# Samsung/tf-fast-rnnt

Hardware: AMD Instinct MI355X
Metric: rnnt_loss_pruned_fwd_bwd_throughput (higher is better)
Workload: dtype f32; 1 GPU; c3: rnnt_loss_pruned fwd+bwd step, B=32/GPU T=1000 S=200 C=500 s_range=5, regular, full boundary, first pass rnnt_loss_simple; global_batch=32, am_pruned=broadcast view

## Files before the change

### tf-fast-rnnt_amd/csrc/capi.hip

```cpp
#include "ftr_common.h"
#ifdef FTR_DIAG
#include "../../include/ftr_diag.h"
#endif
#include <stdlib.h>
#include <string.h>

namespace ftr {
namespace {
thread_local char g_err[512] = {0};
#ifdef FTR_DIAG
int g_mi_impl = -1;
#endif

int device_ok() {
  int n = 0;
  hipError_t e = hipGetDeviceCount(&n);
  if (e != hipSuccess || n <= 0) {
    (void)hipGetLastError();
    set_error("no usable HIP device (%s); this library has no CPU path", e == hipSuccess ? "device count is 0" : hipGetErrorString(e));
    return FTR_ERR_NO_DEVICE;
  }
  return FTR_OK;
}

// ... 635 lines not shown
  if (B == 0) return FTR_OK;
  FTR_REQUIRE(gpy && prod && lm_probs && am_probs && d_am && unigram && am_dot && R && (gpx || S == 0) && (symbols || S == 0), "smoothed_logprobs_fused_bwd_am: null pointer");
  int rc = device_ok();
  if (rc != FTR_OK) return rc;
  return simple_fused_bwd_am(gpx, gpy, Scale{scale, scale_stride, scale_mul}, prod, lm_probs, am_probs, symbols, boundary, termination_symbol, combined_scale, direct_scale, unigram, am_dot, am_only_scale, R, d_am, B, T, S, C, modified, reinterpret_cast<hipStream_t>(stream));
}

int ftr_smoothed_logprobs_bwd_w_scaled_f32(const float* gpx, const float* gpy, const float* scale, int scale_stride,
                                           float scale_mul, const float* prod, const int32_t* boundary,
                                           float combined_scale, float* W, float* rsx, float* rsy, int B, int T, int S,
                                           int modified, void* stream) {
  clear_error();
  FTR_REQUIRE(B >= 0 && T >= 1 && S >= 0, "smoothed_logprobs_bwd_w_scaled: bad sizes");
  FTR_REQUIRE(scale_stride == 0 || scale_stride == 1, "smoothed_logprobs_bwd_w_scaled: scale_stride must be 0 or 1");
  if (B == 0) return FTR_OK;
  FTR_REQUIRE(gpy && prod && W && rsx && rsy && (gpx || S == 0), "smoothed_logprobs_bwd_w_scaled: null pointer");
  int rc = device_ok();
  if (rc != FTR_OK) return rc;
  return simple_logprobs_bwd_w(gpx, gpy, Scale{scale, scale_stride, scale_mul}, prod, boundary, W, rsx, rsy, combined_scale, B, T, S, modified, reinterpret_cast<hipStream_t>(stream));
}

int ftr_smoothed_logprobs_bwd_am_scaled_f32(const float* gpx, const float* gpy, const float* scale, int scale_stride,
                                            float scale_mul, const float* damp, const float* am_probs,
                                            const int32_t* symbols, const int32_t* boundary, int termination_symbol,
                                            float direct_scale, const float* unigram, const float* am_dot,
                                            float am_only_scale, float* R, float* d_am, int B, int T, int S, int C,
                                            int modified, void* stream) {
  clear_error();
  FTR_REQUIRE(B >= 0 && T >= 1 && S >= 0 && C >= 1, "smoothed_logprobs_bwd_am_scaled: bad sizes");
  FTR_REQUIRE(termination_symbol >= 0 && termination_symbol < C, "smoothed_logprobs_bwd_am_scaled: bad termination_symbol");
  FTR_REQUIRE(scale_stride == 0 || scale_stride == 1, "smoothed_logprobs_bwd_am_scaled: scale_stride must be 0 or 1");
  if (B == 0) return FTR_OK;
  FTR_REQUIRE(gpy && damp && am_probs && d_am && unigram && am_dot && R && (gpx || S == 0) && (symbols || S == 0), "smoothed_logprobs_bwd_am_scaled: null pointer");
  int rc = device_ok();
  if (rc != FTR_OK) return rc;
  return simple_logprobs_bwd_am(gpx, gpy, Scale{scale, scale_stride, scale_mul}, damp, am_probs, symbols, boundary, termination_symbol, direct_scale, unigram, am_dot, am_only_scale, R, d_am, B, T, S, C, modified, reinterpret_cast<hipStream_t>(stream));
}

int ftr_mutual_information_band_supported(int T, int S, int r) { return mi_band_supported(T, S, r); }

static int pruned_band_fwd_entry(const float* logits, const int32_t* symbols, const int32_t* ranges, const int32_t* boundary,
                                 int termination_symbol, double delay_penalty, float* lse, float* px_band, float* py_band,
                                 int B, int T, int S, int C, int r, int modified, int hat, void* stream) {
  const char* what = hat ? "hat_pruned_band_fwd" : "pruned_band_fwd";
  clear_error();
  FTR_REQUIRE(B >= 0 && T >= 1 && S >= 0 && C >= 1 && r >= 1, "%s: bad sizes", what);
  FTR_REQUIRE(!hat || C >= 2, "%s: C = %d, HAT needs a blank and at least one other symbol", what, C);
  FTR_REQUIRE(termination_symbol >= 0 && termination_symbol < C, "%s: termination_symbol %d not in [0,%d)", what, termination_symbol, C);
  if (B == 0) return FTR_OK;
  FTR_REQUIRE(logits && ranges && lse && px_band && py_band && (symbols || S == 0), "%s: null pointer", what);
  int rc = device_ok();
  if (rc != FTR_OK) return rc;
  hipStream_t st = reinterpret_cast<hipStream_t>(stream);
  rc = lse_rows(logits, lse, (size_t)B * T * r, C, termination_symbol, hat, st);
  if (rc != FTR_OK) return rc;
  return band_gather(logits, symbols, ranges, boundary, lse, termination_symbol, delay_penalty, px_band, py_band, B, T, S, C, r, modified, hat, st);
}

int ftr_pruned_band_fwd_f32(const float* logits, const int32_t* symbols, const int32_t* ranges, const int32_t* boundary,
                            int termination_symbol, double delay_penalty, float* lse, float* px_band, float* py_band,
                            int B, int T, int S, int C, int r, int modified, void* stream) {
  return pruned_band_fwd_entry(logits, symbols, ranges, boundary, termination_symbol, delay_penalty, lse, px_band, py_band, B, T, S, C, r, modified, 0, stream);
}

int ftr_hat_pruned_band_fwd_f32(const float* logits, const int32_t* symbols, const int32_t* ranges, const int32_t* boundary,
                                int termination_symbol, double delay_penalty, float* lse, float* px_band, float* py_band,
                                int B, int T, int S, int C, int r, int modified, void* stream) {
  return pruned_band_fwd_entry(logits, symbols, ranges, boundary, termination_symbol, delay_penalty, lse, px_band, py_band, B, T, S, C, r, modified, 1, stream);
}

int ftr_band_ranges_check_i32(const int32_t* ranges, const int32_t* boundary, int32_t* flags, int B, int T, int r, void* stream) {
  clear_error();
  FTR_REQUIRE(B >= 0 && T >= 0 && r >= 1, "band_ranges_check: bad sizes");
  FTR_REQUIRE(flags && (ranges || B == 0 || T == 0), "band_ranges_check: null pointer");
  int rc = device_ok();
  if (rc != FTR_OK) return rc;
  return band_ranges_check(ranges, boundary, flags, B, T, r, reinterpret_cast<hipStream_t>(stream));
}

int ftr_mutual_information_band_f32(const float* px_band, const float* py_band, const int32_t* ranges,
                                    const int32_t* boundary, float* ans, float* gx_band, float* gy_band, int B, int T,
                                    int S, int r, int modified, void* stream) {
  return ftr_mutual_information_band_ws_f32(px_band, py_band, ranges, boundary, nullptr, 0, ans, gx_band, gy_band, B, T, S, r, modified, stream);
}

size_t ftr_mutual_information_band_workspace_floats(int B, int T, int S, int r) {
  return (B < 0 || T < 1 || S < 0 || r < 1) ? 0 : mi_band_workspace_floats(B, T, S, r);
}

int ftr_mutual_information_band_ws_f32(const float* px_band, const float* py_band, const int32_t* ranges,
                                       const int32_t* boundary, float* workspace, size_t workspace_floats, float* ans,
                                       float* gx_band, float* gy_band, int B, int T, int S, int r, int modified,
                                       void* stream) {
  clear_error();
  FTR_REQUIRE(B >= 0 && T >= 1 && S >= 0 && r >= 1, "mutual_information_band: bad sizes");
  if (B == 0) return FTR_OK;
  FTR_REQUIRE(px_band && py_band && ranges && ans && gx_band && gy_band, "mutual_information_band: null pointer");
  int rc = device_ok();
  if (rc != FTR_OK) return rc;
  return mi_band(px_band, py_band, ranges, boundary, workspace, workspace_floats, ans, gx_band, gy_band, B, T, S, r, modified, reinterpret_cast<hipStream_t>(stream));
}

static int pruned_band_bwd_scaled_entry(const float* logits, const int32_t* symbols, const int32_t* ranges,
                                        const int32_t* boundary, int termination_symbol, const float* lse,
                                        const float* gx_band, const float* gy_band, const float* scale, int scale_stride,
                                        float scale_mul, float* glogits, int B, int T, int S, int C, int r, int modified,
                                        int hat, void* stream) {
  const char* what = hat ? "hat_pruned_band_bwd_scaled" : "pruned_band_bwd_scaled";
  clear_error();
// ... 282 lines not shown
```

### tf-fast-rnnt_amd/csrc/ftr_common.h

```cpp
#pragma once
#include <hip/hip_runtime.h>
#include <stdint.h>
#include <stdio.h>
#include <stdarg.h>
#include "../../include/ftr.h"

namespace ftr {

void set_error(const char* fmt, ...);
void clear_error();

inline int check_launch(const char* what) {
  hipError_t e = hipGetLastError();
  if (e != hipSuccess) {
    set_error("%s: launch failed: %s", what, hipGetErrorString(e));
    return FTR_ERR_LAUNCH;
  }
  return FTR_OK;
}

inline int require_rows_32bit(const char* what, size_t rows) {
  if (rows > 0x7fffffffull) {
    set_error("%s: %zu rows (B*T*s_range) exceed the 2^31 - 1 that the launch grids index", what, rows);
    return FTR_ERR_INVALID_ARG;
// ... 95 lines not shown
  *sp = xb >= 0.0f ? big : small;
  *sn = xb >= 0.0f ? small : big;
}

}

namespace ftr {
int mi_plain_fwd(const float* px, const float* py, const int32_t* boundary, float* p, float* ans, int B, int S, int T, int modified, hipStream_t st);
int mi_plain_bwd(const float* px, const float* py, const int32_t* boundary, const float* p, float* p_grad, float* px_grad, float* py_grad, float* ans_grad, int overwrite, int B, int S, int T, int modified, hipStream_t st);
int mi_bidir_fwd(const float* px, const float* py, const int32_t* boundary, float* ws, size_t ws_floats, int flags, float* ans, int B, int S, int T, int modified, hipStream_t st);
int mi_bidir_bwd(const int32_t* boundary, const float* ws, size_t ws_floats, int flags, float* px_grad, float* py_grad, float* ans_grad, int overwrite, int B, int S, int T, int modified, hipStream_t st, const float* ans = nullptr, float* loss_out = nullptr, int loss_code = 0);
int mi_bidir_ws_init(float* ws, size_t ws_floats, int B, int S, int T, hipStream_t st);
int mi_bidir_status(const float* ws, size_t ws_floats, int B, int S, int T, int* status_host, long long* dirty_host, hipStream_t st);
size_t mi_bidir_workspace_floats(int B, int S, int T);
size_t mi_bidir_handoff_floats(int B, int S, int T);
size_t mi_viterbi_workspace_bytes(int B, int S, int T);
int mi_viterbi(const float* px, const float* py, const int32_t* boundary, void* ws, size_t ws_bytes, float* score, int32_t* frames, int B, int S, int T, int modified, hipStream_t st);
size_t mi_multiblank_workspace_floats(int B, int S, int T);
int mi_multiblank_fwd(const float* px, const float* py, const int32_t* boundary, const int32_t* durations, int D, float* ws, size_t ws_floats, float* ans, int B, int S, int T, hipStream_t st);
int mi_multiblank_bwd(const float* px, const float* py, const int32_t* boundary, const int32_t* durations, int D, float* ws, size_t ws_floats, const float* ans_grad, float* px_grad, float* py_grad, int B, int S, int T, hipStream_t st);
int multiblank_logprobs_fwd(const float* logits, const int32_t* symbols, const int32_t* ranges, const int32_t* boundary, int blank, const int32_t* big_ids, const int32_t* durations, int D, double sigma, double delay_penalty, float* lse, float* px, float* py, int B, int T, int S, int C, int r, hipStream_t st);
int multiblank_logprobs_bwd(const float* logits, const int32_t* symbols, const int32_t* ranges, const int32_t* boundary, int blank, const int32_t* big_ids, const int32_t* durations, int D, const float* lse, const float* gpx, const float* gpy, Scale scale, float* glogits, int B, int T, int S, int C, int r, hipStream_t st);
size_t mi_tdt_workspace_floats(int B, int S, int T);
int mi_tdt_fwd(const float* px, const float* py, const int32_t* boundary, const int32_t* token_durations, int Dx, const int32_t* blank_durations, int Dy, float* ws, size_t ws_floats, float* ans, int B, int S, int T, hipStream_t st);
int mi_tdt_bwd(const float* px, const float* py, const int32_t* boundary, const int32_t* token_durations, int Dx, const int32_t* blank_durations, int Dy, float* ws, size_t ws_floats, const float* ans_grad, float* px_grad, float* py_grad, int B, int S, int T, hipStream_t st);
int tdt_logprobs_fwd(const float* logits, const int32_t* symbols, const int32_t* ranges, const int32_t* boundary, int blank, const int32_t* durations, int N, double sigma, double delay_penalty, float* lse_tok, float* lse_dur, float* px, float* py, int B, int T, int S, int C, int r, hipStream_t st);
int tdt_logprobs_bwd(const float* logits, const int32_t* symbols, const int32_t* ranges, const int32_t* boundary, int blank, const int32_t* durations, int N, const float* lse_tok, const float* lse_dur, const float* gpx, const float* gpy, Scale scale, float* glogits, int B, int T, int S, int C, int r, hipStream_t st);
int cummin_i32(const int32_t* in, int32_t* out, int rows, int cols, hipStream_t st);
int prune_ranges(const float* px_grad, const float* py_grad, const int32_t* boundary, int32_t* ranges, int32_t* s_begin, int B, int S, int T, int T1, int r, hipStream_t st);
int do_pruning(const float* am, const float* lm, const int32_t* ranges, float* am_p, float* lm_p, int B, int T, int S1, int C, int r, hipStream_t st);
size_t do_pruning_bwd_workspace_bytes(int B, int T, int S1, int C, int r);
int do_pruning_bwd_ws(const float* g_am_p, const float* g_lm_p, const int32_t* ranges, float* d_am, float* d_lm, int B, int T, int S1, int C, int r, void* ws, size_t ws_bytes, hipStream_t st);
int do_pruning_bwd(const float* g_am_p, const float* g_lm_p, const int32_t* ranges, float* d_am, float* d_lm, int B, int T, int S1, int C, int r, hipStream_t st);
int pruned_logprobs_fwd(const float* logits, const int32_t* symbols, const int32_t* ranges, const int32_t* boundary, int blank, double delay_penalty, float* lse, float* px, float* py, int B, int T, int S, int C, int r, int modified, int hat, hipStream_t st);
int pruned_logprobs_bwd(const float* logits, const int32_t* symbols, const int32_t* ranges, const int32_t* boundary, int blank, const float* lse, const float* gpx, const float* gpy, Scale scale, float* glogits, int B, int T, int S, int C, int r, int modified, int hat, hipStream_t st);
int simple_rowmax_exp(const float* x, float* probs, float* rowmax, float* rowsum, const float* dotvec, float* dot, size_t rows, int C, hipStream_t st);
int simple_rowmax_exp_pair(const float* x1, float* probs1, float* rowmax1, size_t rows1, const float* x2, float* probs2, float* rowmax2, size_t rows2, int C, hipStream_t st);
int simple_rowdot(const float* x, const float* v, float* dot, size_t rows, int C, hipStream_t st);
size_t simple_colsum_workspace_floats(size_t rows, int C);
int simple_colsum_weighted(const float* x, const float* w, float* out, float* ws, size_t ws_floats, size_t rows, int C, hipStream_t st);
int simple_logprobs_fwd(const float* am, const float* lm, const int32_t* symbols, const float* prod, const float* am_max, const float* lm_max, const int32_t* boundary, int blank, double delay_penalty, const float* lmonly_norm, const float* amonly_norm, const float* ulog, float cs, float ls, float as, float* px, float* py, int B, int T, int S, int C, int modified, hipStream_t st);
int simple_logprobs_bwd_w(const float* gpx, const float* gpy, Scale scale, const float* prod, const int32_t* boundary, float* W, float* rsx, float* rsy, float cs, int B, int T, int S, int modified, hipStream_t st);
int simple_logprobs_bwd_am(const float* gpx, const float* gpy, Scale scale, const float* damp, const float* am_probs, const int32_t* symbols, const int32_t* boundary, int blank, float kdir, const float* uvec, const float* amdot, float as, float* Rout, float* d_am, int B, int T, int S, int C, int modified, hipStream_t st);
int simple_logprobs_bwd_lm(const float* dlmp, const float* lm_probs, const int32_t* symbols, const float* rsx, const float* rsy, int blank, float kdir, const float* arow, const float* invsum, const float* gu, float* d_lm, int B, int S, int C, hipStream_t st);
int simple_fused_supported(int C);
int simple_fused_bwd_supported(int T, int C);
int normalizer_gemm(int kind, const float* x, const float* y, float* out, int B, int T, int S1, int C, hipStream_t st);
int normalizer_gemm_choice(int kind, int B, int T, int S1, int C, int* solution, float* us, float* us_default, int* candidates);
int normalizer_gemm_set_choice(int kind, int B, int T, int S1, int C, int solution);
int simple_fused_fwd(const float* am, const float* lm, const int32_t* symbols, const float* am_probs, const float* lm_probs, const float* am_max, const float* lm_max, const int32_t* boundary, int blank, double delay_penalty, const float* lmonly_norm, const float* amonly_norm, const float* ulog, float cs, float ls, float as, float* px, float* py, float* prod_out, int B, int T, int S, int C, int modified, hipStream_t st);
int simple_fused_bwd_am(const float* gpx, const float* gpy, Scale scale, const float* prod, const float* lm_probs, const float* am_probs, const int32_t* symbols, const int32_t* boundary, int blank, float cs, float kdir, const float* uvec, const float* amdot, float as, float* Rout, float* d_am, int B, int T, int S, int C, int modified, hipStream_t st);
int negated_reduce(const float* ans, int B, int reduction, float* out, hipStream_t st);
int lse_rows(const float* logits, float* lse, size_t rows, int C, int blank, int hat, hipStream_t st);
int mi_band_supported(int T, int S, int r);
int band_ranges_check(const int32_t* ranges, const int32_t* boundary, int* flags, int B, int T, int r, hipStream_t st);
int band_gather(const float* logits, const int32_t* symbols, const int32_t* ranges, const int32_t* boundary, const float* lse, int blank, double delay_penalty, float* pxb, float* pyb, int B, int T, int S, int C, int r, int modified, int hat, hipStream_t st);
size_t mi_band_workspace_floats(int B, int T, int S, int r);
int mi_band_seg_supported(int T, int S, int r);
size_t mi_band_seg_workspace_floats(int B, int T, int S, int r);
int mi_band_seg(const float* pxb, const float* pyb, const int32_t* ranges, const int32_t* boundary, float* ws, size_t ws_floats, float* ans, float* gxb, float* gyb, int B, int T, int S, int r, int modified, hipStream_t st);
int mi_band(const float* pxb, const float* pyb, const int32_t* ranges, const int32_t* boundary, float* ws, size_t ws_floats, float* ans, float* gxb, float* gyb, int B, int T, int S, int r, int modified, hipStream_t st);
int band_grad_banded(const float* logits, const int32_t* symbols, const int32_t* ranges, const int32_t* boundary, int blank, const float* lse, const float* gxb, const float* gyb, Scale scale, float* glogits, int B, int T, int S, int C, int r, int modified, int hat, hipStream_t st);
int selftest(hipStream_t st, int* result_dev);
int debug_stamps(unsigned long long* out16);
int debug_trace(unsigned long long* out, int n);
}
```

### tf-fast-rnnt_amd/csrc/prune.hip

```cpp
#include "ftr_common.h"
#include <cstdlib>
#include <limits.h>

namespace ftr {
namespace {

__device__ __forceinline__ int wave_incl_min_scan(int v, int lane) {
#pragma unroll
  for (int off = 1; off < 64; off <<= 1) {
    const int t = __shfl_up(v, off, 64);
    if (lane >= off) v = min(v, t);
  }
  return v;
}

__global__ void cummin_kernel(const int32_t* __restrict__ in, int32_t* __restrict__ out, int rows, int cols) {
  const int lane = threadIdx.x & 63;
  const int row = blockIdx.x * (blockDim.x >> 6) + (threadIdx.x >> 6);
  if (row >= rows) return;
  const int32_t* src = in + (size_t)row * cols;
  int32_t* dst = out + (size_t)row * cols;
  int carry = INT_MAX;
  for (int c0 = 0; c0 < cols; c0 += 64) {
    const int c = c0 + lane;
// ... 147 lines not shown
  int best = 0;
  float bestv = 0.0f;
  float nv[2][CHK], xv[2][CHK];
  auto fetch = [&](int c0, float (&n)[CHK], float (&x)[CHK]) {
#pragma unroll
    for (int u = 0; u < CHK; ++u) {
      const int s0 = c0 + u;
      n[u] = (s0 + 1 < nwin) ? pyc[(size_t)(s0 + R) * T] : 0.0f;
      x[u] = (s0 > 0 && s0 < nwin) ? pxc[(size_t)(s0 - 1) * T1] : 0.0f;
    }
  };
  auto consume = [&](int c0, const float (&n)[CHK], const float (&x)[CHK]) {
#pragma unroll
    for (int u = 0; u < CHK; ++u) {
      const int s0 = c0 + u;
      const float g = (u < R) ? carry[u < R ? u : 0] : n[u >= R ? u - R : 0];
      if (s0 < nwin) {
        const float blk = lead - lag;
        const float fin = blk - x[u];
        if (s0 == 0 || fin > bestv) { best = s0; bestv = fin; }
        if (s0 + 1 < nwin) {
          lead = lead + n[u];
          lag = lag + g;
        }
      }
    }
#pragma unroll
    for (int i = 0; i < R; ++i) carry[i] = n[CHK - R + i];
  };
  fetch(0, nv[0], xv[0]);
  for (int c0 = 0; c0 < nwin; c0 += 2 * CHK) {
    if (c0 + CHK < nwin) fetch(c0 + CHK, nv[1], xv[1]);
    consume(c0, nv[0], xv[0]);
    if (c0 + CHK < nwin) {
      if (c0 + 2 * CHK < nwin) fetch(c0 + 2 * CHK, nv[0], xv[0]);
      consume(c0 + CHK, nv[1], xv[1]);
    }
  }
  const int se = boundary[4 * b + 2], te = boundary[4 * b + 3];
  int pad = se - R + 1;
  if (pad < 0) pad = 0;
  s_begin[(size_t)b * T + t] = (t < te - 1) ? best : pad;
}

__device__ __forceinline__ int wave_incl_suffix_min(int v, int lane) {
#pragma unroll
  for (int off = 1; off < 64; off <<= 1) {
    const int t = __shfl_down(v, off, 64);
    if (lane + off < 64) v = min(v, t);
  }
  return v;
}

__global__ void prune_adjust_kernel(const int32_t* __restrict__ s_begin, int32_t* __restrict__ ranges, int B,
                                    int T, int r_out, int r_con) {
  const int lane = threadIdx.x & 63;
  const int b = blockIdx.x * (blockDim.x >> 6) + (threadIdx.x >> 6);
  if (b >= B) return;
  constexpr int PER = 16, SB = 64 * PER;
  const int32_t* x = s_begin + (size_t)b * T;
  int carry1 = INT_MAX, carry2 = INT_MAX;
  for (int base = ((T - 1) / SB) * SB; base >= 0; base -= SB) {
    const int t0 = base + lane * PER;
    int v[PER];
#pragma unroll
    for (int i = 0; i < PER; ++i) v[i] = (t0 + i < T) ? x[t0 + i] : INT_MAX;
#pragma unroll
    for (int i = PER - 2; i >= 0; --i) v[i] = min(v[i], v[i + 1]);
    int incl = wave_incl_suffix_min(v[0], lane);
    int right = __shfl_down(incl, 1, 64);
    right = (lane == 63) ? carry1 : min(right, carry1);
    carry1 = min(__shfl(incl, 0, 64), carry1);
#pragma unroll
    for (int i = 0; i < PER; ++i) {
      const int t = t0 + i;
      v[i] = (t < T) ? -(min(v[i], right) - (r_con - 1) * t) : INT_MAX;
    }
#pragma unroll
    for (int i = PER - 2; i >= 0; --i) v[i] = min(v[i], v[i + 1]);
    incl = wave_incl_suffix_min(v[0], lane);
    right = __shfl_down(incl, 1, 64);
    right = (lane == 63) ? carry2 : min(right, carry2);
    carry2 = min(__shfl(incl, 0, 64), carry2);
#pragma unroll
    for (int i = 0; i < PER; ++i) {
      const int t = t0 + i;
      if (t < T) {
        const int z = max(min(v[i], right), 0);
        const int sb = -(z - (r_con - 1) * t);
        int32_t* dst = ranges + ((size_t)b * T + t) * r_out;
        for (int k = 0; k < r_out; ++k) dst[k] = sb + k;
      }
    }
  }
}

template <bool VEC>
__global__ __launch_bounds__(128) void do_pruning_kernel(const float* __restrict__ am, const float* __restrict__ lm,
                                                         const int32_t* __restrict__ ranges, float* __restrict__ am_p,
                                                         float* __restrict__ lm_p, int T, int S1, int C, int r) {
  const bool copy_am = am_p != nullptr;
  size_t bt = blockIdx.x;
  if ((gridDim.x & 7u) == 0) bt = (size_t)(blockIdx.x & 7u) * (gridDim.x >> 3) + (blockIdx.x >> 3);
  const size_t b = bt / T;
  const int32_t* rg = ranges + bt * r;
  const float* lmb = lm + b * S1 * C;
  float* ao = am_p + bt * r * C;
  float* lo = lm_p + bt * r * C;
  if (VEC) {
    const int n4 = C >> 2;
    const f4u* arow = reinterpret_cast<const f4u*>(am + bt * C);
    for (int c4 = threadIdx.x; c4 < n4; c4 += 128) {
      f4 a = {0.0f, 0.0f, 0.0f, 0.0f};
      if (copy_am) a = arow[c4];
      for (int k0 = 0; k0 < r; k0 += 8) {
        f4 l[8];
#pragma unroll
        for (int u = 0; u < 8; ++u)
          if (k0 + u < r) l[u] = reinterpret_cast<const f4u*>(lmb + (size_t)min(max(rg[k0 + u], 0), S1 - 1) * C)[c4];
#pragma unroll
        for (int u = 0; u < 8; ++u)
          if (k0 + u < r) {
            if (copy_am) __builtin_nontemporal_store(a, reinterpret_cast<f4u*>(ao + (size_t)(k0 + u) * C) + c4);
            __builtin_nontemporal_store(l[u], reinterpret_cast<f4u*>(lo + (size_t)(k0 + u) * C) + c4);
          }
      }
    }
  } else {
    for (int c = threadIdx.x; c < C; c += 128) {
      const float a = copy_am ? am[bt * C + c] : 0.0f;
      for (int k = 0; k < r; ++k) {
        if (copy_am) ao[(size_t)k * C + c] = a;
        lo[(size_t)k * C + c] = lmb[(size_t)min(max(rg[k], 0), S1 - 1) * C + c];
      }
    }
  }
}

template <bool VEC>
__global__ void do_pruning_bwd_am_kernel(const float* __restrict__ g_am_p, float* __restrict__ d_am, int C, int r,
                                         size_t total) {
  const int per_row = VEC ? (C >> 2) : C;
  for (size_t i = (size_t)blockIdx.x * blockDim.x + threadIdx.x; i < total; i += (size_t)gridDim.x * blockDim.x) {
    const size_t bt = i / per_row;
    const int c = (int)(i - bt * per_row);
// ... 392 lines not shown
  const int threads = 256;
  if ((C & 3) == 0) {
    const size_t total = (size_t)B * T * (C >> 2);
    hipLaunchKernelGGL(do_pruning_bwd_am_kernel<true>, dim3((unsigned)((total + threads - 1) / threads)), dim3(threads), 0, st, g_am_p, d_am, C, r, total);
  } else {
    const size_t total = (size_t)B * T * C;
    hipLaunchKernelGGL(do_pruning_bwd_am_kernel<false>, dim3((unsigned)((total + threads - 1) / threads)), dim3(threads), 0, st, g_am_p, d_am, C, r, total);
  }
  int rc = check_launch("do_pruning_bwd_am");
  if (rc != FTR_OK) return rc;
  const size_t lds = sizeof(int) * (size_t)T * r;
  if (lds > 150 * 1024) { set_error("do_pruning_bwd: T*s_range = %d too large for the LDS row list", T * r); return FTR_ERR_UNSUPPORTED; }
  const bool vec = (C & 3) == 0;
  if (lds > 64 * 1024) {
    hipError_t e = vec ? hipFuncSetAttribute(reinterpret_cast<const void*>(do_pruning_bwd_lm_kernel<true>), hipFuncAttributeMaxDynamicSharedMemorySize, (int)lds)
                       : hipFuncSetAttribute(reinterpret_cast<const void*>(do_pruning_bwd_lm_kernel<false>), hipFuncAttributeMaxDynamicSharedMemorySize, (int)lds);
    if (e != hipSuccess) { set_error("do_pruning_bwd: cannot reserve LDS: %s", hipGetErrorString(e)); return FTR_ERR_LAUNCH; }
  }
  if (vec) hipLaunchKernelGGL(do_pruning_bwd_lm_kernel<true>, dim3(S1, B), dim3(64), lds, st, g_lm_p, ranges, d_lm, T, S1, C, r);
  else hipLaunchKernelGGL(do_pruning_bwd_lm_kernel<false>, dim3(S1, B), dim3(64), lds, st, g_lm_p, ranges, d_lm, T, S1, C, r);
  return check_launch("do_pruning_bwd_lm");
}

int cummin_i32(const int32_t* in, int32_t* out, int rows, int cols, hipStream_t st) {
  if (rows == 0 || cols == 0) return FTR_OK;
  const int waves_per_block = 4;
  hipLaunchKernelGGL(cummin_kernel, dim3((rows + waves_per_block - 1) / waves_per_block),
                     dim3(64 * waves_per_block), 0, st, in, out, rows, cols);
  return check_launch("cummin_i32");
}

int prune_ranges(const float* px_grad, const float* py_grad, const int32_t* boundary, int32_t* ranges,
                 int32_t* s_begin, int B, int S, int T, int T1, int r, hipStream_t st) {
  if (B == 0 || T == 0) return FTR_OK;
  const int threads = 64;
  const dim3 grid((T + threads - 1) / threads, B);
#define FTR_ARGMAX_ONCE(R) case R: hipLaunchKernelGGL(prune_argmax_once_kernel<R>, grid, dim3(threads), 0, st, px_grad, py_grad, boundary, s_begin, B, S, T, T1); break;
  const int nwin = S + 1 - r + 1;
  if (nwin > ftr::kSplitQ && (size_t)((T + 63) / 64) * B <= 768) {
    const int nc = (nwin + ftr::kSplitQ - 1) / ftr::kSplitQ;
    const int nw = nc < 8 ? nc : 8;
    hipLaunchKernelGGL(prune_argmax_split_kernel, dim3((T + 63) / 64, B), dim3(64 * nw), 0, st, px_grad, py_grad, boundary, s_begin, B, S, T, T1, r);
  } else
  switch (r) {
    FTR_ARGMAX_ONCE(1) FTR_ARGMAX_ONCE(2) FTR_ARGMAX_ONCE(3) FTR_ARGMAX_ONCE(4) FTR_ARGMAX_ONCE(5) FTR_ARGMAX_ONCE(6)
    FTR_ARGMAX_ONCE(7) FTR_ARGMAX_ONCE(8) FTR_ARGMAX_ONCE(9) FTR_ARGMAX_ONCE(10) FTR_ARGMAX_ONCE(11) FTR_ARGMAX_ONCE(12)
    FTR_ARGMAX_ONCE(13) FTR_ARGMAX_ONCE(14) FTR_ARGMAX_ONCE(15) FTR_ARGMAX_ONCE(16)
    default: hipLaunchKernelGGL(prune_argmax_kernel, grid, dim3(threads), 0, st, px_grad, py_grad, boundary, s_begin, B, S, T, T1, r);
  }
#undef FTR_ARGMAX_ONCE
  int rc = check_launch("prune_argmax");
  if (rc != FTR_OK) return rc;
  const int r_con = (T1 == T) ? 2 : r;
  hipLaunchKernelGGL(prune_adjust_kernel, dim3(B), dim3(64), 0, st, s_begin, ranges, B, T, r, r_con);
  return check_launch("prune_adjust");
}

int do_pruning(const float* am, const float* lm, const int32_t* ranges, float* am_p, float* lm_p, int B, int T, int S1,
               int C, int r, hipStream_t st) {
  const size_t frames = (size_t)B * T;
  if (frames == 0 || C == 0 || r == 0) return FTR_OK;
  { const int rc32 = require_rows_32bit("do_pruning", frames * (size_t)r); if (rc32 != FTR_OK) return rc32; }
  if ((C & 3) == 0) hipLaunchKernelGGL(do_pruning_kernel<true>, dim3((unsigned)frames), dim3(128), 0, st, am, lm, ranges, am_p, lm_p, T, S1, C, r);
  else hipLaunchKernelGGL(do_pruning_kernel<false>, dim3((unsigned)frames), dim3(128), 0, st, am, lm, ranges, am_p, lm_p, T, S1, C, r);
  return check_launch("do_pruning");
}

size_t do_pruning_bwd_workspace_bytes(int B, int T, int S1, int C, int r) {
  if ((C & 3) != 0 || (size_t)B * T * C == 0 || r <= 0) return 0;
  const int seg = ftr::seg_frames(B, T);
  const size_t nseg = (size_t)(T + seg - 1) / seg;
  const size_t partial = sizeof(float) * (size_t)B * nseg * (2 * (size_t)r) * C;
  return partial + sizeof(int4) * (size_t)B * nseg;
}

int do_pruning_bwd_ws(const float* g_am_p, const float* g_lm_p, const int32_t* ranges, float* d_am, float* d_lm,
                      int B, int T, int S1, int C, int r, void* ws, size_t ws_bytes, hipStream_t st) {
  if ((size_t)B * T * C == 0) return FTR_OK;
  if ((C & 3) != 0 || r <= 0) return do_pruning_bwd(g_am_p, g_lm_p, ranges, d_am, d_lm, B, T, S1, C, r, st);
  const size_t need = do_pruning_bwd_workspace_bytes(B, T, S1, C, r);
  if (!ws || ws_bytes < need || (reinterpret_cast<uintptr_t>(ws) & 15) != 0) {
    set_error("do_pruning_bwd_ws: workspace of %zu bytes (16-byte aligned) required, got %zu", need, ws_bytes);
    return FTR_ERR_INVALID_ARG;
  }
  const int seg = ftr::seg_frames(B, T);
  const int nseg = (T + seg - 1) / seg;
  float* partial = reinterpret_cast<float*>(ws);
  int4* meta = reinterpret_cast<int4*>(partial + (size_t)B * nseg * (2 * (size_t)r) * C);
  const size_t lds = sizeof(int) * (size_t)seg;
  if (r > ftr::kSegMaxR || lds > 60 * 1024 || (size_t)B * nseg * (2 * (size_t)r) >= 0x7fffffffull || (size_t)B * T * r >= 0x7fffffffull)
    return do_pruning_bwd(g_am_p, g_lm_p, ranges, d_am, d_lm, B, T, S1, C, r, st);
  const bool fuse = (g_am_p == g_lm_p);
  if (!fuse) {
    const size_t total = (size_t)B * T * (C >> 2);
    hipLaunchKernelGGL(ftr::do_pruning_bwd_am_kernel<true>, dim3((unsigned)((total + 255) / 256)), dim3(256), 0, st, g_am_p, d_am, C, r, total);
    int rc = check_launch("do_pruning_bwd_am");
    if (rc != FTR_OK) return rc;
  }
#define FTR_SEG(R) case R: \
    if (fuse) hipLaunchKernelGGL((ftr::do_pruning_bwd_seg_kernel<R, true>), dim3(nseg, B), dim3(128), lds, st, g_lm_p, ranges, d_am, d_lm, partial, meta, T, S1, C, seg); \
    else hipLaunchKernelGGL((ftr::do_pruning_bwd_seg_kernel<R, false>), dim3(nseg, B), dim3(128), lds, st, g_lm_p, ranges, d_am, d_lm, partial, meta, T, S1, C, seg); \
    break;
  switch (r) {
    FTR_SEG(1) FTR_SEG(2) FTR_SEG(3) FTR_SEG(4) FTR_SEG(5) FTR_SEG(6) FTR_SEG(7) FTR_SEG(8)
    FTR_SEG(9) FTR_SEG(10) FTR_SEG(11) FTR_SEG(12) FTR_SEG(13) FTR_SEG(14) FTR_SEG(15) FTR_SEG(16)
  }
#undef FTR_SEG
// ... 9 lines not shown
```

### tf-fast-rnnt_amd/csrc/pruned_logprobs.hip

```cpp
#include "ftr_common.h"

namespace ftr {
namespace {

__device__ __forceinline__ float wave_max(float v) { return wave_max_dpp(v); }
__device__ __forceinline__ float wave_sum(float v) { return wave_sum_dpp(v); }

template <int NQ, bool HAT>
__global__ __launch_bounds__(256) void lse_rows_reg_kernel(const float* __restrict__ logits, float* __restrict__ lse,
                                                           size_t rows, int C, int blank) {
  const int lane = threadIdx.x & 63;
  const size_t rowi = (size_t)blockIdx.x * (blockDim.x >> 6) + (threadIdx.x >> 6);
  if (rowi >= rows) return;
  const size_t row = rows - 1 - rowi;
  const int n4 = C >> 2;
  const f4 ninf = {-INFINITY, -INFINITY, -INFINITY, -INFINITY};
  const f4u* x4 = reinterpret_cast<const f4u*>(logits + row * C);
  f4 v[NQ];
#pragma unroll
  for (int q = 0; q < NQ; ++q) {
    const int i = lane + 64 * q;
    v[q] = (i < n4) ? (f4)x4[i] : ninf;
    if (HAT) {
#pragma unroll
      for (int e = 0; e < 4; ++e) v[q][e] = (4 * i + e == blank) ? -INFINITY : v[q][e];
    }
  }
  float m = -INFINITY;
#pragma unroll
  for (int q = 0; q < NQ; ++q) m = fmaxf(fmaxf(m, fmaxf(v[q][0], v[q][1])), fmaxf(v[q][2], v[q][3]));
  m = wave_max(m);
  float sum = 0.0f;
#pragma unroll
  for (int q = 0; q < NQ; ++q) {
    if (lane + 64 * q < n4)
      sum += __expf(v[q][0] - m) + __expf(v[q][1] - m) + __expf(v[q][2] - m) + __expf(v[q][3] - m);
  }
  sum = wave_sum(sum);
  if (lane == 0) lse[row] = m + __logf(sum);
}

template <bool VEC, bool HAT>
__global__ void lse_rows_kernel(const float* __restrict__ logits, float* __restrict__ lse, size_t rows, int C, int blank) {
  const int lane = threadIdx.x & 63;
  const size_t row = (size_t)blockIdx.x * (blockDim.x >> 6) + (threadIdx.x >> 6);
  if (row >= rows) return;
  const float* x = logits + row * C;
  float m = -INFINITY;
  if (VEC) {
    const f4u* x4 = reinterpret_cast<const f4u*>(x);
    const int n4 = C >> 2;
    for (int i = lane; i < n4; i += 64) {
      f4 v = x4[i];
      if (HAT) {
#pragma unroll
        for (int e = 0; e < 4; ++e) v[e] = (4 * i + e == blank) ? -INFINITY : v[e];
      }
      m = fmaxf(fmaxf(m, fmaxf(v[0], v[1])), fmaxf(v[2], v[3]));
    }
    m = wave_max(m);
    float s = 0.0f;
    for (int i = lane; i < n4; i += 64) {
      f4 v = x4[i];
      if (HAT) {
#pragma unroll
        for (int e = 0; e < 4; ++e) v[e] = (4 * i + e == blank) ? -INFINITY : v[e];
      }
      s += __expf(v[0] - m) + __expf(v[1] - m) + __expf(v[2] - m) + __expf(v[3] - m);
    }
    s = wave_sum(s);
    if (lane == 0) lse[row] = m + __logf(s);
  } else {
    for (int i = lane; i < C; i += 64) m = fmaxf(m, (HAT && i == blank) ? -INFINITY : x[i]);
    m = wave_max(m);
    float s = 0.0f;
    for (int i = lane; i < C; i += 64) s += __expf(((HAT && i == blank) ? -INFINITY : x[i]) - m);
    s = wave_sum(s);
    if (lane == 0) lse[row] = m + __logf(s);
  }
}

template <bool MOD, bool HAT>
__global__ void band_to_lattice_kernel(const float* __restrict__ logits, const int32_t* __restrict__ symbols,
                                       const int32_t* __restrict__ ranges, const int32_t* __restrict__ boundary,
                                       const float* __restrict__ lse, int blank, double delay_penalty,
                                       float* __restrict__ px, float* __restrict__ py, int T, int S, int C, int r) {
  const int t = blockIdx.x * blockDim.x + threadIdx.x;
  const int s = blockIdx.y, b = blockIdx.z;
  const int T1 = MOD ? T : T + 1;
  if (t >= T1 && t >= T) return;
  const int te = boundary ? boundary[4 * b + 3] : T;
  float vx = -INFINITY, vy = -INFINITY;
// ... 102 lines not shown
          val = gy * sn - gx * sp;
        } else {
          val += gy;
        }
      }
      g[c] = val;
    }
  }
}

__global__ __launch_bounds__(256) void negated_reduce_kernel(const float* __restrict__ ans, int B, int reduction,
                                                             float* __restrict__ out) {
  __shared__ float red[4];
  if (reduction == 0) {
    for (int b = threadIdx.x; b < B; b += 256) out[b] = -ans[b];
    return;
  }
  float s = 0.0f;
  for (int b = threadIdx.x; b < B; b += 256) s += ans[b];
  s = wave_sum(s);
  if ((threadIdx.x & 63) == 0) red[threadIdx.x >> 6] = s;
  __syncthreads();
  if (threadIdx.x == 0) {
    const float t = (red[0] + red[1]) + (red[2] + red[3]);
    out[0] = (reduction == 1) ? -(t / (float)B) : -t;
  }
}
}

int negated_reduce(const float* ans, int B, int reduction, float* out, hipStream_t st) {
  hipLaunchKernelGGL(negated_reduce_kernel, dim3(1), dim3(256), 0, st, ans, B, reduction, out);
  return check_launch("negated_reduce");
}

template <bool HAT>
static void lse_rows_launch(const float* logits, float* lse, size_t rows, int C, int blank, hipStream_t st) {
  const int wpb = 4;
  const unsigned blocks = (unsigned)((rows + wpb - 1) / wpb);
  if ((C & 3) == 0 && C <= 256) hipLaunchKernelGGL((lse_rows_reg_kernel<1, HAT>), dim3(blocks), dim3(64 * wpb), 0, st, logits, lse, rows, C, blank);
  else if ((C & 3) == 0 && C <= 512) hipLaunchKernelGGL((lse_rows_reg_kernel<2, HAT>), dim3(blocks), dim3(64 * wpb), 0, st, logits, lse, rows, C, blank);
  else if ((C & 3) == 0 && C <= 1024) hipLaunchKernelGGL((lse_rows_reg_kernel<4, HAT>), dim3(blocks), dim3(64 * wpb), 0, st, logits, lse, rows, C, blank);
  else if ((C & 3) == 0 && C <= 2048) hipLaunchKernelGGL((lse_rows_reg_kernel<8, HAT>), dim3(blocks), dim3(64 * wpb), 0, st, logits, lse, rows, C, blank);
  else if ((C & 3) == 0) hipLaunchKernelGGL((lse_rows_kernel<true, HAT>), dim3(blocks), dim3(64 * wpb), 0, st, logits, lse, rows, C, blank);
  else hipLaunchKernelGGL((lse_rows_kernel<false, HAT>), dim3(blocks), dim3(64 * wpb), 0, st, logits, lse, rows, C, blank);
}
int lse_rows(const float* logits, float* lse, size_t rows, int C, int blank, int hat, hipStream_t st) {
  if (rows == 0) return FTR_OK;
  { const int rc32 = require_rows_32bit("lse_rows", rows); if (rc32 != FTR_OK) return rc32; }
  if (hat) lse_rows_launch<true>(logits, lse, rows, C, blank, st);
  else lse_rows_launch<false>(logits, lse, rows, C, blank, st);
  return check_launch("lse_rows");
}

int pruned_logprobs_fwd(const float* logits, const int32_t* symbols, const int32_t* ranges,
                        const int32_t* boundary, int blank, double delay_penalty, float* lse, float* px,
                        float* py, int B, int T, int S, int C, int r, int modified, int hat, hipStream_t st) {
  const size_t rows = (size_t)B * T * r;
  if (rows == 0) return FTR_OK;
  { const int rc32 = require_rows_32bit("pruned_logprobs_fwd", rows); if (rc32 != FTR_OK) return rc32; }
  int rc = lse_rows(logits, lse, rows, C, blank, hat, st);
  if (rc != FTR_OK) return rc;
  const int threads = 256;
  const dim3 grid((T + 1 + threads - 1) / threads, S + 1, B);
#define FTR_LAUNCH_BL(MODV, HATV) hipLaunchKernelGGL((band_to_lattice_kernel<MODV, HATV>), grid, dim3(threads), 0, st, \
    logits, symbols, ranges, boundary, lse, blank, delay_penalty, px, py, T, S, C, r)
  if (modified) { if (hat) FTR_LAUNCH_BL(true, true); else FTR_LAUNCH_BL(true, false); }
  else { if (hat) FTR_LAUNCH_BL(false, true); else FTR_LAUNCH_BL(false, false); }
#undef FTR_LAUNCH_BL
  return check_launch("band_to_lattice");
}

int pruned_logprobs_bwd(const float* logits, const int32_t* symbols, const int32_t* ranges,
                        const int32_t* boundary, int blank, const float* lse, const float* gpx,
                        const float* gpy, Scale scale, float* glogits, int B, int T, int S, int C,
                        int r, int modified, int hat, hipStream_t st) {
  const size_t rows = (size_t)B * T * r;
  if (rows == 0) return FTR_OK;
  { const int rc32 = require_rows_32bit("pruned_logprobs_bwd", rows); if (rc32 != FTR_OK) return rc32; }
  const int wpb = 4;
  const unsigned blocks = (unsigned)((rows + wpb - 1) / wpb);
  const bool vec = (C & 3) == 0;
#define FTR_LAUNCH_BG(MODV, VECV, HATV) hipLaunchKernelGGL((band_grad_kernel<MODV, VECV, HATV>), dim3(blocks), dim3(64 * wpb), 0, st, \
    logits, symbols, ranges, boundary, lse, gpx, gpy, scale, blank, glogits, rows, T, S, C, r)
#define FTR_LAUNCH_BGV(MODV, HATV) do { if (vec) FTR_LAUNCH_BG(MODV, true, HATV); else FTR_LAUNCH_BG(MODV, false, HATV); } while (0)
  if (modified) { if (hat) FTR_LAUNCH_BGV(true, true); else FTR_LAUNCH_BGV(true, false); }
  else { if (hat) FTR_LAUNCH_BGV(false, true); else FTR_LAUNCH_BGV(false, false); }
#undef FTR_LAUNCH_BGV
#undef FTR_LAUNCH_BG
  return check_launch("band_grad");
}

namespace {

struct MbCols { int id[8]; int d[8]; int D; };

__device__ __forceinline__ bool mb_is_big_blank(const MbCols& mc, int c) {
  bool hit = false;
  for (int j = 1; j < mc.D; ++j) hit |= (c == mc.id[j]);
  return hit;
}

__global__ void mb_to_lattice_kernel(const float* __restrict__ logits, const int32_t* __restrict__ symbols,
                                     const int32_t* __restrict__ ranges, const int32_t* __restrict__ boundary,
                                     const float* __restrict__ lse, const MbCols mc, float sigma, double delay_penalty,
                                     float* __restrict__ px, float* __restrict__ py, int T, int S, int C, int r) {
  const int t = blockIdx.x * blockDim.x + threadIdx.x;
// ... 155 lines not shown
```

Baseline: 24000 utterances/s.

## Fuse band logprob gather into LSE row kernel; parallelize prune range adjust

The pruned band forward now computes the row log-sum-exp and the px/py band gathers in one kernel. It picks the blank and symbol logits from registers already loaded for the reduction, which removes a second launch and a second read of the logits. Row indices are decoded with precomputed magic-number division, and rows are walked in reverse, likely to reuse cache lines the previous kernel left warm. Separately, the prune range adjust kernel moves from one 64-thread wave per batch to up to 1024 threads per batch, with a cross-wave suffix-min through shared memory and coalesced range writes staged in LDS. This adds block-wide syncs, more shared memory and more complex code.

```diff
diff --git a/tf-fast-rnnt_amd/csrc/capi.hip b/tf-fast-rnnt_amd/csrc/capi.hip
--- a/tf-fast-rnnt_amd/csrc/capi.hip
+++ b/tf-fast-rnnt_amd/csrc/capi.hip
@@ -711,9 +711,7 @@
   int rc = device_ok();
   if (rc != FTR_OK) return rc;
   hipStream_t st = reinterpret_cast<hipStream_t>(stream);
-  rc = lse_rows(logits, lse, (size_t)B * T * r, C, termination_symbol, hat, st);
-  if (rc != FTR_OK) return rc;
-  return band_gather(logits, symbols, ranges, boundary, lse, termination_symbol, delay_penalty, px_band, py_band, B, T, S, C, r, modified, hat, st);
+  return pruned_band_logprobs_fwd(logits, symbols, ranges, boundary, termination_symbol, delay_penalty, lse, px_band, py_band, B, T, S, C, r, modified, hat, st);
 }
 
 int ftr_pruned_band_fwd_f32(const float* logits, const int32_t* symbols, const int32_t* ranges, const int32_t* boundary,
diff --git a/tf-fast-rnnt_amd/csrc/ftr_common.h b/tf-fast-rnnt_amd/csrc/ftr_common.h
--- a/tf-fast-rnnt_amd/csrc/ftr_common.h
+++ b/tf-fast-rnnt_amd/csrc/ftr_common.h
@@ -171,6 +171,7 @@
 int simple_fused_bwd_am(const float* gpx, const float* gpy, Scale scale, const float* prod, const float* lm_probs, const float* am_probs, const int32_t* symbols, const int32_t* boundary, int blank, float cs, float kdir, const float* uvec, const float* amdot, float as, float* Rout, float* d_am, int B, int T, int S, int C, int modified, hipStream_t st);
 int negated_reduce(const float* ans, int B, int reduction, float* out, hipStream_t st);
 int lse_rows(const float* logits, float* lse, size_t rows, int C, int blank, int hat, hipStream_t st);
+int pruned_band_logprobs_fwd(const float* logits, const int32_t* symbols, const int32_t* ranges, const int32_t* boundary, int blank, double delay_penalty, float* lse, float* pxb, float* pyb, int B, int T, int S, int C, int r, int modified, int hat, hipStream_t st);
 int mi_band_supported(int T, int S, int r);
 int band_ranges_check(const int32_t* ranges, const int32_t* boundary, int* flags, int B, int T, int r, hipStream_t st);
 int band_gather(const float* logits, const int32_t* symbols, const int32_t* ranges, const int32_t* boundary, const float* lse, int blank, double delay_penalty, float* pxb, float* pyb, int B, int T, int S, int C, int r, int modified, int hat, hipStream_t st);
diff --git a/tf-fast-rnnt_amd/csrc/prune.hip b/tf-fast-rnnt_amd/csrc/prune.hip
--- a/tf-fast-rnnt_amd/csrc/prune.hip
+++ b/tf-fast-rnnt_amd/csrc/prune.hip
@@ -223,25 +223,41 @@
   return v;
 }
 
-__global__ void prune_adjust_kernel(const int32_t* __restrict__ s_begin, int32_t* __restrict__ ranges, int B,
-                                    int T, int r_out, int r_con) {
-  const int lane = threadIdx.x & 63;
-  const int b = blockIdx.x * (blockDim.x >> 6) + (threadIdx.x >> 6);
-  if (b >= B) return;
-  constexpr int PER = 16, SB = 64 * PER;
+constexpr int kAdjPer = 4;
+__global__ __launch_bounds__(1024) void prune_adjust_kernel(const int32_t* __restrict__ s_begin, int32_t* __restrict__ ranges,
+                                                            int T, int r_out, int r_con) {
+  __shared__ int wmin[2][16];
+  __shared__ int sb_sh[1024 * kAdjPer];
+  constexpr int PER = kAdjPer;
+  const int tid = threadIdx.x, lane = tid & 63, wave = tid >> 6, nw = blockDim.x >> 6;
+  const int b = blockIdx.x;
+  const int SB = blockDim.x * PER;
   const int32_t* x = s_begin + (size_t)b * T;
   int carry1 = INT_MAX, carry2 = INT_MAX;
+  auto right_of = [&](int incl, const int* wm, int& carry) {
+    int right = __shfl_down(incl, 1, 64);
+    if (lane == 63) right = INT_MAX;
+    int tot = INT_MAX;
+    for (int w = 0; w < nw; ++w) {
+      const int m = wm[w];
+      tot = min(tot, m);
+      if (w > wave) right = min(right, m);
+    }
+    right = min(right, carry);
+    carry = min(carry, tot);
+    return right;
+  };
   for (int base = ((T - 1) / SB) * SB; base >= 0; base -= SB) {
-    const int t0 = base + lane * PER;
+    const int t0 = base + tid * PER;
     int v[PER];
 #pragma unroll
     for (int i = 0; i < PER; ++i) v[i] = (t0 + i < T) ? x[t0 + i] : INT_MAX;
 #pragma unroll
     for (int i = PER - 2; i >= 0; --i) v[i] = min(v[i], v[i + 1]);
     int incl = wave_incl_suffix_min(v[0], lane);
-    int right = __shfl_down(incl, 1, 64);
-    right = (lane == 63) ? carry1 : min(right, carry1);
-    carry1 = min(__shfl(incl, 0, 64), carry1);
+    if (lane == 0) wmin[0][wave] = incl;
+    __syncthreads();
+    int right = right_of(incl, wmin[0], carry1);
 #pragma unroll
     for (int i = 0; i < PER; ++i) {
       const int t = t0 + i;
@@ -250,18 +266,23 @@
 #pragma unroll
     for (int i = PER - 2; i >= 0; --i) v[i] = min(v[i], v[i + 1]);
     incl = wave_incl_suffix_min(v[0], lane);
-    right = __shfl_down(incl, 1, 64);
-    right = (lane == 63) ? carry2 : min(right, carry2);
-    carry2 = min(__shfl(incl, 0, 64), carry2);
+    if (lane == 0) wmin[1][wave] = incl;
+    __syncthreads();
+    right = right_of(incl, wmin[1], carry2);
 #pragma unroll
     for (int i = 0; i < PER; ++i) {
       const int t = t0 + i;
       if (t < T) {
         const int z = max(min(v[i], right), 0);
-        const int sb = -(z - (r_con - 1) * t);
-        int32_t* dst = ranges + ((size_t)b * T + t) * r_out;
-        for (int k = 0; k < r_out; ++k) dst[k] = sb + k;
-      }
+        sb_sh[tid * PER + i] = -(z - (r_con - 1) * t);
+      }
+    }
+    __syncthreads();
+    const int n = min(SB, T - base) * r_out;
+    int32_t* dst = ranges + ((size_t)b * T + base) * r_out;
+    for (int i = tid; i < n; i += blockDim.x) {
+      const int q = i / r_out;
+      dst[i] = sb_sh[q] + (i - q * r_out);
     }
   }
 }
@@ -760,7 +781,9 @@
   int rc = check_launch("prune_argmax");
   if (rc != FTR_OK) return rc;
   const int r_con = (T1 == T) ? 2 : r;
-  hipLaunchKernelGGL(prune_adjust_kernel, dim3(B), dim3(64), 0, st, s_begin, ranges, B, T, r, r_con);
+  const int adj_want = ((T + kAdjPer - 1) / kAdjPer + 63) / 64 * 64;
+  const int adj_threads = adj_want < 1024 ? adj_want : 1024;
+  hipLaunchKernelGGL(prune_adjust_kernel, dim3(B), dim3(adj_threads), 0, st, s_begin, ranges, T, r, r_con);
   return check_launch("prune_adjust");
 }
 
diff --git a/tf-fast-rnnt_amd/csrc/pruned_logprobs.hip b/tf-fast-rnnt_amd/csrc/pruned_logprobs.hip
--- a/tf-fast-rnnt_amd/csrc/pruned_logprobs.hip
+++ b/tf-fast-rnnt_amd/csrc/pruned_logprobs.hip
@@ -38,6 +38,90 @@
   }
   sum = wave_sum(sum);
   if (lane == 0) lse[row] = m + __logf(sum);
+}
+
+struct Div31 { unsigned mul; int shift; };
+inline Div31 div31(unsigned d) {
+  if (d <= 1) return Div31{0u, 0};
+  int l = 0;
+  while ((1ull << l) < d) ++l;
+  return Div31{(unsigned)((1ull << (31 + l)) / d + 1), l - 1};
+}
+__device__ __forceinline__ unsigned div31_apply(unsigned i, const Div31 m) { return m.mul ? (__umulhi(i, m.mul) >> m.shift) : i; }
+
+template <int NQ>
+__device__ __forceinline__ float row_pick(const f4 (&v)[NQ], int c) {
+  const int i = c >> 2, e = c & 3;
+  float x = 0.0f;
+#pragma unroll
+  for (int q = 0; q < NQ; ++q)
+#pragma unroll
+    for (int ee = 0; ee < 4; ++ee) x = ((i >> 6) == q && e == ee) ? v[q][ee] : x;
+  return __builtin_bit_cast(float, __builtin_amdgcn_readlane(__builtin_bit_cast(int, x), i & 63));
+}
+
+template <int NQ, bool HAT, bool MOD>
+__global__ __launch_bounds__(256) void lse_rows_band_kernel(const float* __restrict__ logits, const int32_t* __restrict__ symbols,
+                                                            const int32_t* __restrict__ ranges, const int32_t* __restrict__ boundary,
+                                                            int blank, double delay_penalty, float* __restrict__ lse,
+                                                            float* __restrict__ pxb, float* __restrict__ pyb, unsigned rows,
+                                                            int T, int S, int C, int r, const Div31 div_r, const Div31 div_T) {
+  const int lane = threadIdx.x & 63;
+  const unsigned rowi = blockIdx.x * (blockDim.x >> 6) + __builtin_amdgcn_readfirstlane(threadIdx.x >> 6);
+  if (rowi >= rows) return;
+  const unsigned row = rows - 1 - rowi;
+  const int n4 = C >> 2;
+  const f4 ninf = {-INFINITY, -INFINITY, -INFINITY, -INFINITY};
+  const f4u* x4 = reinterpret_cast<const f4u*>(logits + (size_t)row * C);
+  f4 v[NQ];
+#pragma unroll
+  for (int q = 0; q < NQ; ++q) {
+    const int i = lane + 64 * q;
+    v[q] = (i < n4) ? (f4)x4[i] : ninf;
+  }
+  const unsigned bt = div31_apply(row, div_r);
+  const int k = (int)(row - bt * (unsigned)r);
+  const int b = (int)div31_apply(bt, div_T);
+  const int t = (int)(bt - (unsigned)b * (unsigned)T);
+  const int s = ranges[(size_t)bt * r] + k;
+  const int te = boundary ? boundary[4 * b + 3] : T;
+  const bool sok = s >= 0 && s <= S;
+  int c = blank;
+  if (sok && s < S) c = min(max(symbols[(size_t)b * S + s], 0), C - 1);
+  const float xb = row_pick<NQ>(v, blank), xs = row_pick<NQ>(v, c);
+  if (HAT) {
+#pragma unroll
+    for (int q = 0; q < NQ; ++q)
+#pragma unroll
+      for (int e = 0; e < 4; ++e) v[q][e] = (4 * (lane + 64 * q) + e == blank) ? -INFINITY : v[q][e];
+  }
+  float m = -INFINITY;
+#pragma unroll
+  for (int q = 0; q < NQ; ++q) m = fmaxf(fmaxf(m, fmaxf(v[q][0], v[q][1])), fmaxf(v[q][2], v[q][3]));
+  m = wave_max(m);
+  float sum = 0.0f;
+#pragma unroll
+  for (int q = 0; q < NQ; ++q) {
+    if (lane + 64 * q < n4)
+      sum += __expf(v[q][0] - m) + __expf(v[q][1] - m) + __expf(v[q][2] - m) + __expf(v[q][3] - m);
+  }
+  sum = wave_sum(sum);
+  if (lane == 0) {
+    const float l = m + __logf(sum);
+    lse[row] = l;
+    float vy = -INFINITY, vx = -INFINITY;
+    if (sok) {
+      if (HAT) hat_logprobs(xb, xs, l, c == blank, &vx, &vy);
+      else vy = xb - l;
+      if (s < S) {
+        if (!HAT) vx = xs - l;
+        if (!MOD && t == te) vx = -INFINITY;
+        if (delay_penalty > 0.0) vx += (float)((((double)te - 1.0) / 2.0 - (double)t) * delay_penalty);
+      }
+    }
+    pxb[row] = vx;
+    pyb[row] = vy;
+  }
 }
 
 template <bool VEC, bool HAT>
@@ -246,6 +330,39 @@
   return check_launch("lse_rows");
 }
 
+template <bool HAT, bool MOD>
+static void lse_rows_band_launch(const float* logits, const int32_t* symbols, const int32_t* ranges, const int32_t* boundary,
+                                 int blank, double delay_penalty, float* lse, float* pxb, float* pyb, size_t rows, int T, int S,
+                                 int C, int r, hipStream_t st) {
+  const int wpb = 4;
+  const unsigned blocks = (unsigned)((rows + wpb - 1) / wpb);
+  const Div31 dr = div31((unsigned)r), dT = div31((unsigned)T);
+#define FTR_LAUNCH_LB(NQV) hipLaunchKernelGGL((lse_rows_band_kernel<NQV, HAT, MOD>), dim3(blocks), dim3(64 * wpb), 0, st, logits, symbols, \
+    ranges, boundary, blank, delay_penalty, lse, pxb, pyb, (unsigned)rows, T, S, C, r, dr, dT)
+  if (C <= 256) FTR_LAUNCH_LB(1);
+  else if (C <= 512) FTR_LAUNCH_LB(2);
+  else if (C <= 1024) FTR_LAUNCH_LB(4);
+  else FTR_LAUNCH_LB(8);
+#undef FTR_LAUNCH_LB
+}
+int pruned_band_logprobs_fwd(const float* logits, const int32_t* symbols, const int32_t* ranges, const int32_t* boundary,
+                             int blank, double delay_penalty, float* lse, float* pxb, float* pyb, int B, int T, int S, int C,
+                             int r, int modified, int hat, hipStream_t st) {
+  const size_t rows = (size_t)B * T * r;
+  if (rows == 0) return FTR_OK;
+  { const int rc32 = require_rows_32bit("pruned_band_fwd", rows); if (rc32 != FTR_OK) return rc32; }
+  if ((C & 3) != 0 || C > 2048) {
+    const int rc = lse_rows(logits, lse, rows, C, blank, hat, st);
+    if (rc != FTR_OK) return rc;
+    return band_gather(logits, symbols, ranges, boundary, lse, blank, delay_penalty, pxb, pyb, B, T, S, C, r, modified, hat, st);
+  }
+#define FTR_LAUNCH_LBV(HATV, MODV) lse_rows_band_launch<HATV, MODV>(logits, symbols, ranges, boundary, blank, delay_penalty, lse, pxb, pyb, rows, T, S, C, r, st)
+  if (hat) { if (modified) FTR_LAUNCH_LBV(true, true); else FTR_LAUNCH_LBV(true, false); }
+  else { if (modified) FTR_LAUNCH_LBV(false, true); else FTR_LAUNCH_LBV(false, false); }
+#undef FTR_LAUNCH_LBV
+  return check_launch("lse_rows_band");
+}
+
 int pruned_logprobs_fwd(const float* logits, const int32_t* symbols, const int32_t* ranges,
                         const int32_t* boundary, int blank, double delay_penalty, float* lse, float* px,
                         float* py, int B, int T, int S, int C, int r, int modified, int hat, hipStream_t st) {
```

After: 24100 utterances/s, median of 4. About the same (+0.4%).
